# justinkay/aldi

Hardware: AMD Instinct MI355X
Metric: images/sec (student+teacher ALDI step), R50-FPN 1333x800 (higher is better)
Workload: dtype bf16

## Files before the change

### aldi_amd/csrc/elementwise.hip

```cpp
#include "common.h"
#include <stdlib.h>

namespace {

template <typename T>
__global__ void dgrad_weights_kernel(const float* __restrict__ w, const float* __restrict__ scale, T* __restrict__ wt,
                                     int Cout, int KH, int KW, int Cin) {
    long total = (long)Cout * KH * KW * Cin;
    for (long i = blockIdx.x * (long)blockDim.x + threadIdx.x; i < total; i += (long)gridDim.x * blockDim.x) {
        int co = (int)(i % Cout);
        long r = i / Cout;
        int kw = (int)(r % KW); r /= KW;
        int kh = (int)(r % KH);
        int ci = (int)(r / KH);
        float v = w[(((long)co * KH + (KH - 1 - kh)) * KW + (KW - 1 - kw)) * Cin + ci];
        if (scale) v *= scale[co];
        Elem<T>::st(wt + i, v);
    }
}

template <typename T>
__global__ __launch_bounds__(256) void dgrad_weights_batch_kernel(const aldi_dgw_item* __restrict__ items, int n_items) {
    __shared__ float tl[32][33];
    const int tile = blockIdx.x;
// ... 502 lines not shown
        p[i] = w;
        if (pc) Elem<T>::st(pc + i, w);
    }
}

template <typename T>
__global__ void ema_kernel(float* __restrict__ t, const float* __restrict__ s, T* __restrict__ tc, long n, long nc, float one_minus_alpha, float alpha,
                           int copy_only) {
    const long n4 = ((reinterpret_cast<uintptr_t>(t) | reinterpret_cast<uintptr_t>(s)) & 15) == 0 ? n >> 2 : 0;
    for (long q = blockIdx.x * (long)blockDim.x + threadIdx.x; q < n4; q += (long)gridDim.x * blockDim.x) {
        const float4 sv = reinterpret_cast<const float4*>(s)[q];
        float4 v = sv;
        if (!copy_only) {
            const float4 tv = reinterpret_cast<const float4*>(t)[q];
            v.x = sv.x * one_minus_alpha + tv.x * alpha; v.y = sv.y * one_minus_alpha + tv.y * alpha;
            v.z = sv.z * one_minus_alpha + tv.z * alpha; v.w = sv.w * one_minus_alpha + tv.w * alpha;
        }
        reinterpret_cast<float4*>(t)[q] = v;
        if (tc) {
            const long i = q << 2;
            if (i < nc) Elem<T>::st(tc + i, v.x);
            if (i + 1 < nc) Elem<T>::st(tc + i + 1, v.y);
            if (i + 2 < nc) Elem<T>::st(tc + i + 2, v.z);
            if (i + 3 < nc) Elem<T>::st(tc + i + 3, v.w);
        }
    }
    for (long i = (n4 << 2) + blockIdx.x * (long)blockDim.x + threadIdx.x; i < n; i += (long)gridDim.x * blockDim.x) {
        float v = copy_only ? s[i] : s[i] * one_minus_alpha + t[i] * alpha;
        t[i] = v;
        if (tc && i < nc) Elem<T>::st(tc + i, v);
    }
}

__global__ void bn_fold_kernel(const float* __restrict__ w, const float* __restrict__ b, const float* __restrict__ mean,
                               const float* __restrict__ var, float* __restrict__ scale, float* __restrict__ shift, int C, float eps) {
    int i = blockIdx.x * blockDim.x + threadIdx.x;
    if (i < C) {
        float sc = w[i] * (1.0f / sqrtf(var[i] + eps));
        scale[i] = sc;
        shift[i] = b[i] - mean[i] * sc;
    }
}

static inline int nblocks(long n, int per = 256, int cap = 16384) {
    long b = (n + per - 1) / per;
    return (int)(b < 1 ? 1 : (b > cap ? cap : b));
}

}

#define DISPATCH_T(dtype, KERNEL, grid, block, st, ...)                                              \
    do {                                                                                             \
        if ((dtype) == ALDI_BF16) hipLaunchKernelGGL(KERNEL<bf16_t>, grid, block, 0, st, __VA_ARGS__); \
        else if ((dtype) == ALDI_F32) hipLaunchKernelGGL(KERNEL<float>, grid, block, 0, st, __VA_ARGS__); \
        else return aldi_set_error_msg(ALDI_ERR_ARG, #KERNEL ": bad dtype");                         \
        ALDI_CHECK_LAUNCH();                                                                         \
    } while (0)

extern "C" int aldi_stem_forward(const aldi_stem_args* a, aldi_stream_t stream) {
    if (!a || !a->img || !a->w || !a->y || a->N < 1 || a->N > ALDI_MAX_IMAGES) return aldi_set_error_msg(ALDI_ERR_ARG, "stem_forward: bad args");
    StemDev d;
    d.img = a->img; d.w = a->w; d.scale = a->scale; d.shift = a->shift; d.y = a->y;
    d.N = a->N; d.Hs = a->Hs; d.Ws = a->Ws; d.Hc = a->Hc; d.Wc = a->Wc;
    for (int i = 0; i < a->N; ++i) { d.h[i] = a->h[i]; d.wd[i] = a->w_img[i]; }
    for (int c = 0; c < 3; ++c) { d.mean[c] = a->mean[c]; d.inv_std[c] = 1.0f / a->std[c]; }
    dim3 grid(cdiv(a->Wc, 16), cdiv(a->Hc, 16), a->N);
// ... 134 lines not shown
extern "C" int aldi_sgd_step(float* p, const float* g, float* buf, void* p_compute, long n, float lr, float momentum, float weight_decay,
                             float grad_scale, int first_step, int dtype, aldi_stream_t stream) {
    if (!p || !g || !buf) return aldi_set_error_msg(ALDI_ERR_ARG, "sgd_step: null pointer");
    hipStream_t st = static_cast<hipStream_t>(stream);
    if (dtype == ALDI_BF16) hipLaunchKernelGGL(sgd_kernel<bf16_t>, dim3(nblocks(n)), dim3(256), 0, st, p, g, buf, (bf16_t*)p_compute, n, lr, momentum, weight_decay, grad_scale, first_step);
    else hipLaunchKernelGGL(sgd_kernel<float>, dim3(nblocks(n)), dim3(256), 0, st, p, g, buf, (float*)nullptr, n, lr, momentum, weight_decay, grad_scale, first_step);
    ALDI_CHECK_LAUNCH();
    return ALDI_OK;
}

extern "C" int aldi_sgd_step_dev(float* p, const float* g, float* buf, void* p_compute, long n, const float* hyper, int dtype, aldi_stream_t stream) {
    if (!p || !g || !buf || !hyper || n <= 0) return aldi_set_error_msg(ALDI_ERR_ARG, "sgd_step_dev: bad args");
    hipStream_t st = static_cast<hipStream_t>(stream);
    if (dtype == ALDI_BF16) hipLaunchKernelGGL(sgd_dev_kernel<bf16_t>, dim3(nblocks(n)), dim3(256), 0, st, p, g, buf, (bf16_t*)p_compute, n, hyper);
    else hipLaunchKernelGGL(sgd_dev_kernel<float>, dim3(nblocks(n)), dim3(256), 0, st, p, g, buf, (float*)nullptr, n, hyper);
    ALDI_CHECK_LAUNCH();
    return ALDI_OK;
}

extern "C" int aldi_ema_update(float* teacher, const float* student, void* teacher_compute, long n, long n_compute, double alpha, int copy_only, int dtype,
                               aldi_stream_t stream) {
    if (!teacher || !student) return aldi_set_error_msg(ALDI_ERR_ARG, "ema_update: null pointer");
    hipStream_t st = static_cast<hipStream_t>(stream);
    const float oma = (float)(1.0 - alpha);
    const float alpha_f = (float)alpha;
    const long nc = teacher_compute ? (n_compute < n ? n_compute : n) : 0;
    const int cap = aldi_tuning().ema_blocks > 0 ? aldi_tuning().ema_blocks : 16384;
    if (dtype == ALDI_BF16) hipLaunchKernelGGL(ema_kernel<bf16_t>, dim3(nblocks(n / 4 + 1, 256, cap)), dim3(256), 0, st, teacher, student, (bf16_t*)teacher_compute, n, nc, oma, alpha_f, copy_only);
    else hipLaunchKernelGGL(ema_kernel<float>, dim3(nblocks(n / 4 + 1, 256, cap)), dim3(256), 0, st, teacher, student, (float*)nullptr, n, 0L, oma, alpha_f, copy_only);
    ALDI_CHECK_LAUNCH();
    return ALDI_OK;
}

extern "C" int aldi_bn_fold(const float* w, const float* b, const float* mean, const float* var, float* scale, float* shift, int C, aldi_stream_t stream) {
    hipLaunchKernelGGL(bn_fold_kernel, dim3(cdiv(C, 256)), dim3(256), 0, static_cast<hipStream_t>(stream), w, b, mean, var, scale, shift, C, 1e-5f);
    ALDI_CHECK_LAUNCH();
    return ALDI_OK;
}

extern "C" int aldi_dgrad_weights_batch(const aldi_dgw_item* items, int n_items, int total_tiles, int dtype, aldi_stream_t stream) {
    if (!items || n_items <= 0 || total_tiles <= 0) return aldi_set_error_msg(ALDI_ERR_ARG, "dgrad_weights_batch: bad args");
    hipStream_t st = static_cast<hipStream_t>(stream);
    if (dtype == ALDI_BF16) hipLaunchKernelGGL(dgrad_weights_batch_kernel<bf16_t>, dim3(total_tiles), dim3(256), 0, st, items, n_items);
    else if (dtype == ALDI_F32) hipLaunchKernelGGL(dgrad_weights_batch_kernel<float>, dim3(total_tiles), dim3(256), 0, st, items, n_items);
    else return aldi_set_error_msg(ALDI_ERR_ARG, "dgrad_weights_batch: bad dtype");
    ALDI_CHECK_LAUNCH();
    return ALDI_OK;
}

extern "C" int aldi_dgrad_weights(const float* w_master, const float* scale, void* wt, int Cout, int KH, int KW, int Cin,
                                  int dtype, aldi_stream_t stream) {
    if (!w_master || !wt) return aldi_set_error_msg(ALDI_ERR_ARG, "dgrad_weights: null pointer");
    long total = (long)Cout * KH * KW * Cin;
    int blocks = (int)((total + 255) / 256);
    if (blocks > 8192) blocks = 8192;
    hipStream_t st = static_cast<hipStream_t>(stream);
    if (dtype == ALDI_BF16) hipLaunchKernelGGL(dgrad_weights_kernel<bf16_t>, dim3(blocks), dim3(256), 0, st, w_master, scale, (bf16_t*)wt, Cout, KH, KW, Cin);
    else hipLaunchKernelGGL(dgrad_weights_kernel<float>, dim3(blocks), dim3(256), 0, st, w_master, scale, (float*)wt, Cout, KH, KW, Cin);
    ALDI_CHECK_LAUNCH();
    return ALDI_OK;
}
```

### aldi_amd/engine.py

```python
from __future__ import annotations

import contextlib
import dataclasses
import inspect
import math
import os
from collections import OrderedDict
from typing import Dict, List, Optional, Sequence, Tuple

import torch

from . import ops
from .arch import FC_DIM, FPN_C, NUM_ANCHORS, POOL, STAGE_BLOCKS, Packed, ParamLayout, pad_to

PIXEL_MEAN = (103.530, 116.280, 123.675)
PIXEL_STD = (1.0, 1.0, 1.0)
ANCHOR_SIZES = (32, 64, 128, 256, 512)
ANCHOR_RATIOS = (0.5, 1.0, 2.0)
STRIDES = (4, 8, 16, 32, 64)
GMAX = 128
RPN_BATCH, RPN_POS_FRAC = 256, 0.5
ROI_BATCH, ROI_POS_FRAC = 512, 0.25
RPN_PRE = (2000, 1000)
RPN_POST = (1000, 1000)
# ... 23 lines not shown
            a, a2 = torch.randperm(n_)[:k_], torch.randperm(17)
            torch.manual_seed(12345)
            b, b2 = fast(n_, k_), torch.randperm(17)
            ok = ok and torch.equal(a, b) and torch.equal(a2, b2)
        torch.set_rng_state(saved)
        _FAST_RANDPERM = ok
    if _FAST_RANDPERM:
        return fast(n, k)
    return torch.randperm(n)[:k]


class Weights:

    def __init__(self, layout: ParamLayout, device, dtype: torch.dtype, trainable: bool):
        self.layout, self.device, self.dtype, self.trainable = layout, device, dtype, trainable
        L = layout
        self.master = torch.zeros(L.n_total, dtype=torch.float32, device=device)
        self.compute = self.master if dtype == torch.float32 else torch.zeros(L.n_weights, dtype=dtype, device=device)
        self.bn_scale = torch.zeros(max(L.bn_channels, 1), dtype=torch.float32, device=device)
        self.bn_shift = torch.zeros(max(L.bn_channels, 1), dtype=torch.float32, device=device)
        self._grad = None
        self._mom = None
        self.first_step = True
        self._wt: Dict[str, torch.Tensor] = {}
        self._wt_keys: List[str] = []
        self._wt_plan = None
        self.wt_epoch = 0
        self._neg1: Dict[int, torch.Tensor] = {}
        self._stem_pk, self._stem_name = None, None
        self.lazy_wt = False
        self._wt_dirty = False
        self._fold_names: List[str] = []
        self._fold_plan = None

    @property
    def grad(self) -> torch.Tensor:
        if self._grad is None:
            self._grad = torch.zeros(self.layout.n_train, dtype=torch.float32, device=self.device)
        return self._grad

    @property
    def mom(self) -> torch.Tensor:
        if self._mom is None:
            self._mom = torch.zeros(self.layout.n_train, dtype=torch.float32, device=self.device)
        return self._mom

    def w(self, name: str) -> torch.Tensor:
        p = self.layout.t[name]
        n = p.rows * p.kk * p.kk * p.cin
        return self.compute[p.w_off: p.w_off + n].view(p.wshape)

    def w_master(self, name: str) -> torch.Tensor:
        p = self.layout.t[name]
        n = p.rows * p.kk * p.kk * p.cin
        return self.master[p.w_off: p.w_off + n].view(p.wshape)

    def b(self, name: str) -> Optional[torch.Tensor]:
        p = self.layout.t[name]
        return self.master[p.b_off: p.b_off + p.rows] if p.bias else None

    def scale(self, name: str) -> Optional[torch.Tensor]:
        p = self.layout.t[name]
        return self.bn_scale[p.bn_off: p.bn_off + p.rows] if p.bn else None

    def shift(self, name: str) -> Optional[torch.Tensor]:
        p = self.layout.t[name]
# ... 42 lines not shown
        neg = key.endswith("-")
        key = key[:-1] if neg else key
        flat = key.endswith("@flat")
        name = key[:-len("@flat")] if flat else key
        w = self.w_master(name)
        if flat:
            w = w.view(w.shape[0], 1, 1, -1)
        return w, self._wt_scale(name, neg)

    def _wt_scale(self, name: str, negate: bool):
        if not negate:
            return self.scale(name)
        rows = self.layout.t[name].rows
        if rows not in self._neg1:
            self._neg1[rows] = torch.full((rows,), -1.0, dtype=torch.float32, device=self.device)
        return self._neg1[rows]

    def _refresh_wt(self):
        self._wt_dirty = False
        self._wt.clear()
        if not self._wt_keys:
            return
        if self._wt_plan is None:
            self._wt_plan = ops.DgradWeightsPlan([self._wt_source(key) for key in self._wt_keys], self.dtype)
        self._wt_plan.run()
        for key, o in zip(self._wt_keys, self._wt_plan.out):
            self._wt[key] = o

    def load_state_dict(self, sd: Dict[str, torch.Tensor]):
        missing = [k for k in self.layout.state_dict_keys() if k not in sd]
        if missing:
            raise KeyError(f"missing keys in state_dict: {missing[:5]}{'...' if len(missing) > 5 else ''}")
        self.master.copy_(self.layout.pack(sd).to(self.device))
        self.refresh()

    def state_dict(self) -> "OrderedDict[str, torch.Tensor]":
        return self.layout.unpack(self.master)

    def refresh(self, cast: bool = True):
        L = self.layout
        if L.bn_channels:
            b = L.bn_base
            c = L.bn_channels
            ops.bn_fold(self.master[b:b + c], self.master[b + c:b + 2 * c], self.master[b + 2 * c:b + 3 * c],
                        self.master[b + 3 * c:b + 4 * c], self.bn_scale, self.bn_shift, c)
        if self.dtype != torch.float32 and cast:
            ops.cast_from_f32(self.master[:L.n_weights], self.dtype, out=self.compute)
        if self._stem_pk is not None:
            ops.stem_pack_weights(self.w_master(self._stem_name), out=self._stem_pk)
        if self._fold_plan is not None:
            self._fold_plan.run()
        self._refresh_wt()

    def zero_grad(self):
        self.grad.zero_()
        self._gscale = 1.0

    def scale_grad(self, f: float):
        self._gscale = getattr(self, "_gscale", 1.0) * f

    def sgd_step(self, lr: float, momentum: float = 0.9, weight_decay: float = 1e-4, grad_scale: float = 1.0):
        n = self.layout.n_train
        ops.sgd_step(self.master, self.grad, self.mom, self.compute if self.dtype != torch.float32 else None, n, lr, momentum,
                     weight_decay, grad_scale * getattr(self, "_gscale", 1.0), self.first_step, self.dtype)
        self._after_sgd()

    def _after_sgd(self):
        self.first_step = False
        if self.lazy_wt:
            self._wt_dirty = True
        else:
            self._refresh_wt()

    def sgd_range_dev(self, lo: int, hi: int, hyper: torch.Tensor):
        hi = min(hi, self.layout.n_train)
        if hi > lo:
            ops.sgd_step_dev(self.master, self.grad, self.mom, self.compute if self.dtype != torch.float32 else None, lo, hi, hyper, self.dtype)

    def ema_from(self, student: "Weights", alpha: float, copy_only: bool):
        n = self.layout.n_total
        if self.dtype == torch.bfloat16:
            ops.ema_update(self.master, student.master, self.compute, n, alpha, copy_only, self.dtype, n_compute=self.layout.n_weights)
            self.refresh(cast=False)
        else:
            ops.ema_update(self.master, student.master, None, n, alpha, copy_only, torch.float32)
            self.refresh()


def make_anchors(shapes: Sequence[Tuple[int, int]], device, sizes: Sequence[float] = ANCHOR_SIZES) -> torch.Tensor:
    out = []
    for (h, w), size, stride in zip(shapes, sizes, STRIDES):
        cell = []
        for r in ANCHOR_RATIOS:
            area = size ** 2.0
            aw = math.sqrt(area / r)
            ah = r * aw
            cell.append([-aw / 2.0, -ah / 2.0, aw / 2.0, ah / 2.0])
        cell = torch.tensor(cell, dtype=torch.float32)
# ... 1259 lines not shown
```

### aldi_amd/ops.py

```python
from __future__ import annotations

import ctypes as C
import os
from typing import List, Optional, Sequence

import torch

from . import _lib as L


def dtype_code(t: torch.dtype) -> int:
    if t == torch.float32:
        return L.F32
    if t == torch.bfloat16:
        return L.BF16
    raise TypeError(f"unsupported dtype {t}")


def _p(t: Optional[torch.Tensor]):
    return None if t is None else t.data_ptr()


_RAW_STREAM = getattr(torch._C, "_cuda_getCurrentRawStream", None)

# ... 299 lines not shown
    L.call("aldi_subsample2", _p(x), _p(y), N, H, W_, Cc, 0, dtype_code(x.dtype), stream_ptr())
    return y


def subsample2_bwd(g_small: torch.Tensor, g_big: torch.Tensor) -> None:
    N, H, W_, Cc = g_big.shape
    L.call("aldi_subsample2", _p(g_small), _p(g_big), N, H, W_, Cc, 1, dtype_code(g_big.dtype), stream_ptr())


def upsample2_bwd(g: torch.Tensor, out: torch.Tensor, accumulate: bool) -> None:
    N, Hc, Wc, Cc = out.shape
    assert g.shape == (N, Hc * 2, Wc * 2, Cc)
    L.call("aldi_upsample2_bwd", _p(g), _p(out), N, Hc, Wc, Cc, int(accumulate), dtype_code(g.dtype), stream_ptr())


def upsample2_bwd_chain(g2: torch.Tensor, o3: torch.Tensor, o4: torch.Tensor, o5: torch.Tensor) -> None:
    N, H5, W5, Cc = o5.shape
    assert o4.shape == (N, H5 * 2, W5 * 2, Cc) and o3.shape == (N, H5 * 4, W5 * 4, Cc) and g2.shape == (N, H5 * 8, W5 * 8, Cc)
    L.call("aldi_upsample2_bwd_chain", _p(g2), _p(o3), _p(o4), _p(o5), N, H5, W5, Cc, dtype_code(g2.dtype), stream_ptr())


def add_f32(a: Optional[torch.Tensor], b: Optional[torch.Tensor], out: torch.Tensor, relu_src: Optional[torch.Tensor] = None) -> torch.Tensor:
    L.call("aldi_add_f32", _p(a), _p(b), _p(relu_src), _p(out), out.numel(), dtype_code(out.dtype), stream_ptr())
    return out


def cast_from_f32(src: torch.Tensor, dtype: torch.dtype, out: Optional[torch.Tensor] = None) -> torch.Tensor:
    if out is None:
        out = torch.empty(src.shape, dtype=dtype, device=src.device)
    L.call("aldi_cast_from_f32", _p(src), _p(out), src.numel(), dtype_code(dtype), stream_ptr())
    return out


def sgd_step(p, g, buf, p_compute, n, lr, momentum, weight_decay, grad_scale, first_step, dtype) -> None:
    L.call("aldi_sgd_step", _p(p), _p(g), _p(buf), _p(p_compute), n, lr, momentum, weight_decay, grad_scale, int(first_step),
           dtype_code(dtype), stream_ptr())


def sgd_step_dev(p, g, buf, p_compute, lo: int, hi: int, hyper: torch.Tensor, dtype) -> None:
    pc = None if p_compute is None else p_compute.data_ptr() + lo * p_compute.element_size()
    L.call("aldi_sgd_step_dev", p.data_ptr() + 4 * lo, g.data_ptr() + 4 * lo, buf.data_ptr() + 4 * lo, pc, hi - lo, _p(hyper), dtype_code(dtype), stream_ptr())


def ema_update(teacher, student, teacher_compute, n, alpha, copy_only, dtype, n_compute=None) -> None:
    nc = 0 if teacher_compute is None else (teacher_compute.numel() if n_compute is None else n_compute)
    L.call("aldi_ema_update", _p(teacher), _p(student), _p(teacher_compute), n, nc, alpha, int(copy_only), dtype_code(dtype), stream_ptr())


def bn_fold(w, b, mean, var, scale, shift, Cc) -> None:
    L.call("aldi_bn_fold", _p(w), _p(b), _p(mean), _p(var), _p(scale), _p(shift), Cc, stream_ptr())


def make_geom(shapes: Sequence[Sequence[int]], A: int, Cc: int) -> L.RpnGeom:
    g = L.RpnGeom()
    g.num_levels, g.A, g.C = len(shapes), A, Cc
    off = 0
    for i, (h, w) in enumerate(shapes):
        g.H[i], g.W[i], g.off[i] = h, w, off
        off += h * w * A
    for i in range(len(shapes), L.MAX_LEVELS + 1):
        g.off[i] = off
    return g


def ptrs(ts: Optional[Sequence[Optional[torch.Tensor]]]):
    if ts is None:
        return None
# ... 160 lines not shown
```

### aldi_amd/trainer.py

```python
from __future__ import annotations

import contextlib
import copy
import logging
import os
import time
import weakref
from typing import Callable, Dict, List, NamedTuple, Optional

from collections import OrderedDict

import torch
import torch.distributed as dist

from . import synthetic
from .dataloader import DeviceStrongAugLoader, SyntheticDetectionLoader, WeakStrongDataloader, device_strong_seed
from .distill import build_distiller
from .ema import EMA
from .model import build_aldi

DEBUG = False
debug_dict = {}


# ... 216 lines not shown
        for k, v in out.items():
            if row.keep(k):
                entries.append((f"{k}_{name}", v))
    kept = [(n_, v) for n_, v in entries if not isinstance(v, tuple)]
    masked = [(n_, v[0]) for n_, v in entries if isinstance(v, tuple)]
    vals = {}
    if kept:
        kv = (torch.stack([v for _, v in kept]) / accum).detach()
        vals.update({n_: kv[i] for i, (n_, _) in enumerate(kept)})
    if masked:
        mv = ((torch.stack([v for _, v in masked]) * 0.0) / accum).detach()
        vals.update({n_: mv[i] for i, (n_, _) in enumerate(masked)})
    for n_, _ in entries:
        loss_dict[n_] = loss_dict[n_] + vals[n_] if n_ in loss_dict else vals[n_]
    eng.backward_fused(c, scales)
    model._last_fused = c
    return loss_dict


def _num_classes(cfg) -> int:
    if cfg.MODEL.META_ARCHITECTURE == "DeformableDETR":
        return int(cfg.MODEL.DEFORMABLE_DETR.NUM_CLASSES)
    return int(cfg.MODEL.ROI_HEADS.NUM_CLASSES)


class EngineSGD:
    def __init__(self, model, lr, momentum=0.9, weight_decay=1e-4):
        self.model = model
        self.param_groups = [{"lr": lr, "momentum": momentum, "weight_decay": weight_decay}]

    def zero_grad(self, set_to_none: bool = False):
        self.model.weights.zero_grad()

    def step(self):
        W = self.model.weights
        if getattr(W, "_sgd_applied", False):
            W._sgd_applied = False
            W._after_sgd()
            return
        g = self.param_groups[0]
        W.sgd_step(g["lr"], g["momentum"], g["weight_decay"])

    def state_dict(self):
        W = self.model.weights
        return {"format": "aldi_amd.flat_sgd", "param_groups": [dict(g) for g in self.param_groups],
                "momentum_buffer": None if W._mom is None else W.mom.detach().cpu().clone(), "first_step": bool(W.first_step)}

    def load_state_dict(self, sd):
        W = self.model.weights
        if sd.get("format") != "aldi_amd.flat_sgd":
            logging.getLogger(__name__).warning("optimizer state of a foreign format: momentum restarts from zero")
            return
        for g, h in zip(self.param_groups, sd.get("param_groups", [])):
            g.update({k: v for k, v in h.items() if k in ("momentum", "weight_decay")})
        if sd.get("momentum_buffer") is not None:
            W.mom.copy_(sd["momentum_buffer"].to(W.mom.device))
        W.first_step = bool(sd.get("first_step", sd.get("momentum_buffer") is None))


class EngineAdamW:
    def __init__(self, model, lr, weight_decay=0.1, betas=(0.9, 0.999), lr_decay_rate=None, num_layers=12):
        self.model = model
        self.param_groups = [{"lr": lr, "weight_decay": weight_decay, "betas": betas}]
        self.lr_decay_rate, self.num_layers = lr_decay_rate, num_layers

    def zero_grad(self, set_to_none: bool = False):
        self.model.weights.zero_grad()

    def step(self):
        g = self.param_groups[0]
        kw = {}
        if self.lr_decay_rate is not None:
            kw = dict(lr_decay_rate=self.lr_decay_rate, num_layers=self.num_layers)
# ... 87 lines not shown
        self.last_loss_dict: Dict[str, float] = {}

    @property
    def _data_loader_iter(self):
        if self._data_loader_iter_obj is None:
            self._data_loader_iter_obj = iter(self.data_loader)
        return self._data_loader_iter_obj

    def run_step(self):
        if not self.model.training:
            raise AssertionError("[SimpleTrainer] model was changed to eval mode!")
        t0 = time.perf_counter()
        batch = self._fetch_batch()
        fetch_s = time.perf_counter() - t0
        clear_first = self.zero_grad_before_forward
        if clear_first and self._defers_zero_grad():
            self._zero_pending = True
        elif clear_first:
            self.optimizer.zero_grad()
        if self._defers_sgd():
            self._sgd_pending = True
        result = self.run_model(batch)
        self.__dict__.pop("_sgd_pending", None)
        fused = bool(getattr(self, "_fused_done", False))
        if isinstance(result, torch.Tensor):
            loss_dict, total = {"total_loss": result}, result
        else:
            loss_dict, total = result, (None if fused else sum(result.values()))
        if not clear_first and not fused:
            self.optimizer.zero_grad()
        self.do_backward(total)
        self.after_backward()
        self._write_metrics(loss_dict, fetch_s)
        self.optimizer.step()

    def run_model(self, data):
        return self.model(data)

    def _wants_lookahead(self) -> bool:
        return False

    def _fetch_batch(self):
        if not self._wants_lookahead():
            ahead = self.__dict__.pop("_ahead_batch", None)
            self._next_batch = None
            return ahead if ahead is not None else next(self._data_loader_iter)
        ahead = self.__dict__.pop("_ahead_batch", None)
        batch = ahead if ahead is not None else next(self._data_loader_iter)
        try:
            self._ahead_batch = next(self._data_loader_iter)
        except StopIteration:
            self._ahead_batch = None
        self._next_batch = self._ahead_batch
        return batch

    def _defers_zero_grad(self) -> bool:
        return False

    def _defers_sgd(self) -> bool:
        return False

    def do_backward(self, losses):
        losses.backward()

    def after_backward(self):
        if _data_parallel():
# ... 84 lines not shown
            return False
        chunks = [ls[i:i + bs] for i in range(0, len(ls), bs)]
        if do_distill:
            from .distill import HardDistiller
            from .helpers import foreign_hooks
            d = self.distiller
            if type(d) is not HardDistiller or uw is None or us is None or len(uw) != len(us) or len(us) == 0 or len(us) % bs:
                return False
            if any(foreign_hooks(m.module if hasattr(m, "module") else m, []) for m in (d.student, d.teacher)):
                return False
            chunks += [us[i:i + bs] for i in range(0, len(us), bs)]
        if sum(len(c_) for c_ in chunks) > 16:
            return False
        canvas = {(max(int(b["image"].shape[-2]) for b in c_), max(int(b["image"].shape[-1]) for b in c_)) for c_ in chunks}
        return len({((h + 31) // 32, (w + 31) // 32) for h, w in canvas}) == 1

    def _wants_lookahead(self) -> bool:
        from .engine import RCNN
        model = self.model.module if hasattr(self.model, "module") else self.model
        eng = getattr(model, "engine", None)
        return (bool(self.fused) and (bool(model.cfg.SOLVER.get("PIPELINE_PREFIX", False)) or os.environ.get("ALDI_PIPELINE_PREFIX") == "1") and os.environ.get("ALDI_PIPELINE_PREFIX") != "0"
                and os.environ.get("ALDI_FUSED_LEGACY", "0") != "1" and type(eng) is RCNN and eng.prefix_pipelinable())

    def _defers_zero_grad(self) -> bool:
        from .engine import RCNN
        model = self.model.module if hasattr(self.model, "module") else self.model
        return bool(self.fused) and os.environ.get("ALDI_FUSED_LEGACY", "0") != "1" and type(getattr(model, "engine", None)) is RCNN

    def _defers_sgd(self) -> bool:
        W = getattr(self.model, "weights", None)
        return (self._defers_zero_grad() and isinstance(self.optimizer, EngineSGD) and not _data_parallel() and W is not None
                and not W.first_step and os.environ.get("ALDI_SGD_IN_STEP", "0") == "1")

    def run_model(self, data):
        self._fused_done = False
        pending_ema = self.__dict__.pop("_pending_ema", None)
        if pending_ema is not None and not self._can_fuse(data):
            pending_ema[0].update_weights(self.model, pending_ema[1])
            pending_ema = None
        defer = self.__dict__.pop("_zero_pending", False)
        if defer and not self._can_fuse(data):
            self.optimizer.zero_grad()
            defer = False
        if self._can_fuse(data):
            self._fused_done = True
            if not self.zero_grad_before_forward:
                if self._defers_zero_grad():
                    defer = True
                else:
                    self.optimizer.zero_grad()
            eng = self.model.engine
            reducer = None
            if _data_parallel():
                from .reduce import BucketedReducer, resolve_exchange
                reducer = self._reducer = BucketedReducer(self.model.weights.grad, payload=str(self.model.cfg.SOLVER.get("GRAD_PAYLOAD", "fp32")),
                                                          exchange=resolve_exchange(self.model.cfg.SOLVER.get("GRAD_EXCHANGE", "auto")))
                eng.grad_ready = reducer.ready
            ok = False
            try:
                if os.environ.get("ALDI_FUSED_LEGACY", "0") == "1":
                    out = fused_run_model(self, *data)
                    ok = True
                    return out
                if getattr(self, "_fused_step", None) is None:
                    from .fused_step import FusedStep
                    self._fused_step = FusedStep(self)
                sgd = None
                if self.__dict__.pop("_sgd_pending", False) and reducer is None:
                    g_ = self.optimizer.param_groups[0]
                    sgd = (g_["lr"], g_["momentum"], g_["weight_decay"])
                out = self._fused_step.run(*data, ema=pending_ema, zero_grad=defer, reducer=reducer, sgd=sgd,
                                           next_data=self.__dict__.get("_next_batch") if self._wants_lookahead() else None)
                ok = True
                return out
            finally:
                eng.grad_ready = None
                if not ok:
                    self._reducer = None
        if self._can_fuse_detr(data):
            self._fused_done = True
            return fused_run_model_detr(self, *data)
        return run_model_labeled_unlabeled(self, *data)

    def do_backward(self, losses, override=False):
        if getattr(self, "_fused_done", False):
            return
        if self.backward_at_end or override:
            super().do_backward(losses)


class ALDIAMPTrainer(_ALDITrainer, AMPTrainer):
    pass


class ALDISimpleTrainer(_ALDITrainer, SimpleTrainer):
    pass


class DefaultTrainer:
    def __init__(self, cfg):
        self.cfg = cfg
        model = self.build_model(cfg)
        optimizer = self.build_optimizer(cfg, model)
        data_loader = self.build_train_loader(cfg)
        model = self.create_ddp_model(model, broadcast_buffers=False, cfg=cfg)
        self._trainer = self._create_trainer(cfg, model, data_loader, optimizer)
# ... 128 lines not shown
        total = cfg.SOLVER.IMS_PER_BATCH
        sizes = [int(total * r / sum(ratios)) for r in ratios]
        if sum(sizes) != total:
            raise AssertionError(f"sum(batch_sizes)={sum(sizes)} must equal total_batch_size={total}")
        share = {}
        for part, n in zip(contents, sizes):
            share[part] = max(share.get(part, 0), n)
        labeled_bs = max((n for part, n in share.items() if part.startswith("labeled")), default=0)
        unlabeled_bs = max((n for part, n in share.items() if part.startswith("unlabeled")), default=0)
        batch_contents = contents
        world = dist.get_world_size() if dist.is_available() and dist.is_initialized() else 1
        rank = dist.get_rank() if world > 1 else 0
        syn = cfg.get("SYNTHETIC", {})
        h, w = syn.get("HEIGHT", 800), syn.get("WIDTH", 1333)
        K = _num_classes(cfg)
        fixed = bool(syn.get("FIXED", False))
        labeled_loader = SyntheticDetectionLoader(labeled_bs // world, h, w, K, 1000 + 17 * rank, True, fixed=fixed) if labeled_bs > 0 else None
        unlabeled_loader = SyntheticDetectionLoader(unlabeled_bs // world, h, w, K, 2000 + 17 * rank, False, fixed=fixed) if unlabeled_bs > 0 else None
        if cfg.AUG.get("DEVICE_STRONG", False):
            from .aug import get_strong_augs
            base = max(int(cfg.SEED), 0)
            if labeled_loader is not None:
                labeled_loader = DeviceStrongAugLoader(labeled_loader, get_strong_augs(cfg, True) if "labeled_strong" in contents else None,
                                                       device_strong_seed(base, rank, True))
            if unlabeled_loader is not None:
                unlabeled_loader = DeviceStrongAugLoader(unlabeled_loader, get_strong_augs(cfg, False) if "unlabeled_strong" in contents else None,
                                                         device_strong_seed(base, rank, False))
        return WeakStrongDataloader(labeled_loader, unlabeled_loader, batch_contents)

    def before_step(self):
        super(ALDITrainer, self).before_step()
        if self.cfg.EMA.ENABLED:
            t = self._trainer
            if getattr(t, "fused", False) and os.environ.get("ALDI_FUSED_LEGACY", "0") != "1" and type(t.model.engine).__name__ == "RCNN":
                t._pending_ema = (self.ema, self.iter)
            else:
                self.ema.update_weights(t.model, self.iter)

    @classmethod
    def build_test_loader(cls, cfg, dataset_name):
        syn_ = cfg.get("SYNTHETIC", {})
        h, w = syn_.get("HEIGHT", 800), syn_.get("WIDTH", 1333)
        n, K = int(syn_.get("VAL_IMAGES", 8)), _num_classes(cfg)
        g = torch.Generator().manual_seed(4242)
        batches, records = [], []
        for i in range(n):
            img, inst = synthetic.make_image(h, w, int(torch.randint(5, 21, (1,), generator=g)), K, g)
            batches.append([{"image": img, "image_id": i, "height": h, "width": w}])
            records.append(dict(image_id=i, height=h, width=w,
                                annotations=[dict(bbox=b.tolist(), bbox_mode="XYXY_ABS", category_id=int(c))
                                             for b, c in zip(inst["gt_boxes"], inst["gt_classes"])]))
        return batches, records

    @classmethod
    def build_evaluator(cls, cfg, dataset_name, output_folder=None, dataset_dicts=None):
        from .evaluation import Detectron2COCOEvaluatorAdapter, DeviceCOCOEvaluator
        if output_folder is None:
            output_folder = os.path.join(cfg.OUTPUT_DIR, "inference")
        if cfg.TEST.get("DEVICE_EVAL", False):
            return DeviceCOCOEvaluator(dataset_name, dataset_dicts or [], _num_classes(cfg), output_dir=output_folder)
        return Detectron2COCOEvaluatorAdapter(dataset_name, dataset_dicts or [], _num_classes(cfg), output_dir=output_folder)

    @classmethod
    def test(cls, cfg, model, evaluators=None):
        from .evaluation import inference_on_dataset
        names = list(cfg.DATASETS.TEST) or ["synthetic_val"]
# ... 29 lines not shown
```

### include/aldi_hip.h

```cpp
#ifndef ALDI_HIP_H
#define ALDI_HIP_H
#include <stddef.h>
#include <stdint.h>

#ifdef __cplusplus
extern "C" {
#endif

typedef void* aldi_stream_t;

enum { ALDI_F32 = 0, ALDI_BF16 = 1 };
enum { ALDI_OK = 0, ALDI_ERR_HIP = -1, ALDI_ERR_ARG = -2 };

const char* aldi_last_error(void);
int aldi_version(void);
int aldi_noop(aldi_stream_t stream);

int aldi_set_tuning(const char* name, int value);
int aldi_get_tuning(const char* name, int* value);
int aldi_reset_tuning(void);
const char* aldi_last_dispatch(void);

typedef struct {
    const void* x;
// ... 66 lines not shown
} aldi_fold_item;
int aldi_fold_weights_batch(const aldi_fold_item* items, int n_items, int total_chunks, aldi_stream_t stream);

#define ALDI_MAX_IMAGES 16

typedef struct {
    const uint8_t* img;
    const float* w;
    const float* scale; const float* shift;
    void* y;
    int N, Hs, Ws, Hc, Wc;
    int h[ALDI_MAX_IMAGES], w_img[ALDI_MAX_IMAGES];
    float mean[3], std[3];
    int dtype;
} aldi_stem_args;
int aldi_stem_forward(const aldi_stem_args* a, aldi_stream_t stream);
int aldi_stem_pack_weights(const float* w, void* w_packed, aldi_stream_t stream);
int aldi_stem_pool_forward(const aldi_stem_args* a, const void* w_packed, void* y_pool, aldi_stream_t stream);

int aldi_maxpool3s2(const void* x, void* y, int N, int H, int W, int C, int dtype, aldi_stream_t stream);
int aldi_stage_images(const void* const* images, const int* heights, const int* widths, int n, int C, int Hs, int Ws, void* batch,
                      aldi_stream_t stream);
int aldi_subsample2(const void* x, void* y, int N, int H, int W, int C, int backward, int dtype, aldi_stream_t stream);
int aldi_upsample2_bwd(const void* g, void* out, int N, int Hc, int Wc, int C, int accumulate, int dtype, aldi_stream_t stream);
int aldi_upsample2_bwd_chain(const void* g2, void* o3, void* o4, void* o5, int N, int H5, int W5, int C, int dtype, aldi_stream_t stream);
int aldi_add_f32(const void* a, const float* b, const void* relu_src, void* out, long n, int dtype, aldi_stream_t stream);
int aldi_cast_from_f32(const float* src, void* dst, long n, int dtype, aldi_stream_t stream);

int aldi_sgd_step(float* p, const float* g, float* buf, void* p_compute, long n, float lr, float momentum, float weight_decay,
                  float grad_scale, int first_step, int dtype, aldi_stream_t stream);
int aldi_sgd_step_dev(float* p, const float* g, float* buf, void* p_compute, long n, const float* hyper, int dtype, aldi_stream_t stream);
int aldi_ema_update(float* teacher, const float* student, void* teacher_compute, long n, long n_compute, double alpha, int copy_only, int dtype,
                    aldi_stream_t stream);
int aldi_bn_fold(const float* w, const float* b, const float* mean, const float* var, float* scale, float* shift, int C, aldi_stream_t stream);

#define ALDI_MAX_LEVELS 5
typedef struct {
    int num_levels;
    int A;
    int C;
    int H[ALDI_MAX_LEVELS], W[ALDI_MAX_LEVELS];
    int off[ALDI_MAX_LEVELS + 1];
} aldi_rpn_geom;

int aldi_box_match(const float* boxes, long box_stride_n, const int* box_count, int L,
                   const float* gt_boxes, const int* gt_count, int Gmax, int N,
                   float lo, float hi, int allow_low_quality,
                   float* best_iou, int* best_idx, unsigned* gt_best_scratch, size_t gt_best_bytes, int* labels, aldi_stream_t stream);
size_t aldi_compact_labels_workspace(int L, int N);
int aldi_compact_labels(const int* labels, int L, int N, int bg_label, int* lists, int* counts, void* workspace, aldi_stream_t stream);
int aldi_rpn_apply_sample(int* labels, int L, int N, const int* lists, const int* sel, const int* nsel, int S, aldi_stream_t stream);
int aldi_rpn_loss(const aldi_rpn_geom* gm, float* const* head, float* const* grad, const float* anchors, const int* labels, const int* matched,
                  const float* gt_boxes, const int* gt_count, int Gmax, int N, float inv_norm, float grad_scale_cls, float grad_scale_loc,
                  float* loss2, aldi_stream_t stream);
size_t aldi_rpn_proposals_workspace(int N, int num_levels);
int aldi_rpn_proposals(const aldi_rpn_geom* gm, float* const* head, const float* anchors, const int* img_hw, int N,
                       int pre_nms_topk, int post_nms_topk, float nms_thresh, void* workspace,
                       float* out_boxes, float* out_scores, int* out_count, int* err_flag, aldi_stream_t stream);

size_t aldi_rpn_active_pixels_workspace(const aldi_rpn_geom* gm, int N);
int aldi_rpn_active_pixels(const aldi_rpn_geom* gm, float* const* grad_head, int N, int cap, int* idx, int* count, void* workspace,
                           int* err_flag, aldi_stream_t stream);
int aldi_rpn_sparse_gather(const aldi_rpn_geom* gm, float* const* grad_head, const void* const* hidden, const void* const* feat, int N, int Cf,
                           int cap, const int* idx, const int* count, void* G, void* Tm, void* X9, int dtype, aldi_stream_t stream);
int aldi_rpn_sparse_scatter(const aldi_rpn_geom* gm, void* const* gfeat, const void* Y, int N, int Cf, int cap, const int* idx,
                            const int* count, int dtype, int grad_dtype, aldi_stream_t stream);
// ... 196 lines not shown
```

Baseline: 498.0.

## Fuse SGD step with next iteration's teacher EMA update in one kernel

Adds a state_step kernel that applies SGD momentum to the student master weights, writes the bf16 compute copy, and immediately applies the EMA lerp (or copy) into the teacher master and teacher bf16 copy in the same pass. The trainer rides the next iteration's EMA tick on the optimizer step when the fused path ran, then skips the separate EMA update in before_step. This removes a second full pass over the student weights and one extra kernel launch per iteration. In exchange it adds cross-iteration bookkeeping (tick_applied_for) and guards for eval, checkpoint and last-iteration boundaries.

```diff
diff --git a/aldi_amd/csrc/elementwise.hip b/aldi_amd/csrc/elementwise.hip
--- a/aldi_amd/csrc/elementwise.hip
+++ b/aldi_amd/csrc/elementwise.hip
@@ -558,6 +558,43 @@
     }
 }
 
+template <typename T>
+__global__ __launch_bounds__(256) void state_step_kernel(float* __restrict__ p, float* __restrict__ g, float* __restrict__ buf, T* __restrict__ pc,
+                                                         float* __restrict__ t, T* __restrict__ tc, long n_train, long n_weights, long n_total,
+                                                         float lr, float mu, float wd, float gscale, int first, float one_minus_alpha, float alpha,
+                                                         int copy_only, int clear_grad) {
+    const long n4 = n_total >> 2;
+    for (long q = blockIdx.x * (long)blockDim.x + threadIdx.x; q < n4; q += (long)gridDim.x * blockDim.x) {
+        const long i = q << 2;
+        float w[4];
+        load4(p + i, w);
+        if (i < n_train) {
+            float gv[4], b[4];
+            load4(g + i, gv);
+            if (!first) load4(buf + i, b);
+#pragma unroll
+            for (int k = 0; k < 4; ++k) {
+                const float d = gv[k] * gscale + wd * w[k];
+                b[k] = first ? d : mu * b[k] + d;
+                w[k] = w[k] - lr * b[k];
+            }
+            store4(buf + i, b);
+            store4(p + i, w);
+            store4(pc + i, w);
+            if (clear_grad) *reinterpret_cast<float4*>(g + i) = make_float4(0.f, 0.f, 0.f, 0.f);
+        }
+        float v[4] = {w[0], w[1], w[2], w[3]};
+        if (!copy_only) {
+            float tv[4];
+            load4(t + i, tv);
+#pragma unroll
+            for (int k = 0; k < 4; ++k) v[k] = w[k] * one_minus_alpha + tv[k] * alpha;
+        }
+        store4(t + i, v);
+        if (i < n_weights) store4(tc + i, v);
+    }
+}
+
 __global__ void bn_fold_kernel(const float* __restrict__ w, const float* __restrict__ b, const float* __restrict__ mean,
                                const float* __restrict__ var, float* __restrict__ scale, float* __restrict__ shift, int C, float eps) {
     int i = blockIdx.x * blockDim.x + threadIdx.x;
@@ -758,6 +795,25 @@
     return ALDI_OK;
 }
 
+extern "C" int aldi_state_step(float* p, float* g, float* buf, void* p_compute, float* teacher, void* teacher_compute, long n_train, long n_weights,
+                               long n_total, float lr, float momentum, float weight_decay, float grad_scale, int first_step, double alpha, int copy_only,
+                               int clear_grad, int dtype, aldi_stream_t stream) {
+    if (!p || !g || !buf || !p_compute || !teacher || !teacher_compute) return aldi_set_error_msg(ALDI_ERR_ARG, "state_step: null pointer");
+    if (dtype != ALDI_BF16) return aldi_set_error_msg(ALDI_ERR_ARG, "state_step: bf16 compute copies only");
+    if (n_train < 0 || n_train > n_weights || n_weights > n_total || n_total <= 0 || ((n_train | n_weights | n_total) & 3))
+        return aldi_set_error_msg(ALDI_ERR_ARG, "state_step: need 0 <= n_train <= n_weights <= n_total, each a multiple of 4");
+    if (((reinterpret_cast<uintptr_t>(p) | reinterpret_cast<uintptr_t>(g) | reinterpret_cast<uintptr_t>(buf) | reinterpret_cast<uintptr_t>(teacher)) & 15) ||
+        ((reinterpret_cast<uintptr_t>(p_compute) | reinterpret_cast<uintptr_t>(teacher_compute)) & 7))
+        return aldi_set_error_msg(ALDI_ERR_ARG, "state_step: buffers must be 16-byte aligned (compute copies: 8)");
+    const float oma = (float)(1.0 - alpha);
+    const float alpha_f = (float)alpha;
+    hipLaunchKernelGGL(state_step_kernel<bf16_t>, dim3(nblocks(n_total >> 2)), dim3(256), 0, static_cast<hipStream_t>(stream), p, g, buf, (bf16_t*)p_compute,
+                       teacher, (bf16_t*)teacher_compute, n_train, n_weights, n_total, lr, momentum, weight_decay, grad_scale, first_step, oma, alpha_f,
+                       copy_only, clear_grad);
+    ALDI_CHECK_LAUNCH();
+    return ALDI_OK;
+}
+
 extern "C" int aldi_bn_fold(const float* w, const float* b, const float* mean, const float* var, float* scale, float* shift, int C, aldi_stream_t stream) {
     hipLaunchKernelGGL(bn_fold_kernel, dim3(cdiv(C, 256)), dim3(256), 0, static_cast<hipStream_t>(stream), w, b, mean, var, scale, shift, C, 1e-5f);
     ALDI_CHECK_LAUNCH();
diff --git a/aldi_amd/engine.py b/aldi_amd/engine.py
--- a/aldi_amd/engine.py
+++ b/aldi_amd/engine.py
@@ -79,6 +79,7 @@
         self._wt_dirty = False
         self._fold_names: List[str] = []
         self._fold_plan = None
+        self.tick_applied_for = None
 
     @property
     def grad(self) -> torch.Tensor:
@@ -187,6 +188,7 @@
         if missing:
             raise KeyError(f"missing keys in state_dict: {missing[:5]}{'...' if len(missing) > 5 else ''}")
         self.master.copy_(self.layout.pack(sd).to(self.device))
+        self.tick_applied_for = None
         self.refresh()
 
     def state_dict(self) -> "OrderedDict[str, torch.Tensor]":
@@ -219,6 +221,20 @@
         ops.sgd_step(self.master, self.grad, self.mom, self.compute if self.dtype != torch.float32 else None, n, lr, momentum,
                      weight_decay, grad_scale * getattr(self, "_gscale", 1.0), self.first_step, self.dtype)
         self._after_sgd()
+
+    def sgd_ema_step(self, teacher: "Weights", alpha: float, copy_only: bool, lr: float, momentum: float = 0.9, weight_decay: float = 1e-4,
+                     clear_grad: bool = False):
+        L = self.layout
+        T = teacher.layout
+        if self.dtype != torch.bfloat16 or teacher.dtype != torch.bfloat16 or (L.n_train, L.n_weights, L.n_total) != (T.n_train, T.n_weights, T.n_total):
+            raise ValueError("sgd_ema_step: student and teacher must be bf16 models of the same flat layout")
+        ops.sgd_step(self.master, self.grad, self.mom, self.compute, L.n_train, lr, momentum, weight_decay, getattr(self, "_gscale", 1.0),
+                     self.first_step, self.dtype, teacher=teacher.master, teacher_compute=teacher.compute, n_weights=L.n_weights,
+                     n_total=L.n_total, alpha=alpha, copy_only=copy_only, clear_grad=clear_grad)
+        if clear_grad:
+            self._gscale = 1.0
+        self._after_sgd()
+        teacher.refresh(cast=False)
 
     def _after_sgd(self):
         self.first_step = False
diff --git a/aldi_amd/ops.py b/aldi_amd/ops.py
--- a/aldi_amd/ops.py
+++ b/aldi_amd/ops.py
@@ -355,7 +355,12 @@
     return out
 
 
-def sgd_step(p, g, buf, p_compute, n, lr, momentum, weight_decay, grad_scale, first_step, dtype) -> None:
+def sgd_step(p, g, buf, p_compute, n, lr, momentum, weight_decay, grad_scale, first_step, dtype, *, teacher=None, teacher_compute=None,
+             n_weights=None, n_total=None, alpha=None, copy_only=False, clear_grad=False) -> None:
+    if teacher is not None:
+        L.call("aldi_state_step", _p(p), _p(g), _p(buf), _p(p_compute), _p(teacher), _p(teacher_compute), n, n_weights, n_total, lr, momentum,
+               weight_decay, grad_scale, int(first_step), float(alpha), int(copy_only), int(clear_grad), dtype_code(dtype), stream_ptr())
+        return
     L.call("aldi_sgd_step", _p(p), _p(g), _p(buf), _p(p_compute), n, lr, momentum, weight_decay, grad_scale, int(first_step),
            dtype_code(dtype), stream_ptr())
 
diff --git a/aldi_amd/state_step.py b/aldi_amd/state_step.py
--- /dev/null
+++ b/aldi_amd/state_step.py
@@ -0,0 +1,18 @@
+import os
+
+
+def enabled() -> bool:
+    return os.environ.get("ALDI_STATE_STEP", "1") != "0"
+
+
+def tick_may_ride(it: int, max_iter: int, eval_period: int = 0, checkpoint_period: int = 0) -> bool:
+    if it + 1 >= max_iter:
+        return False
+    for period in (eval_period, checkpoint_period):
+        if period and period > 0 and (it + 1) % period == 0:
+            return False
+    return True
+
+
+def tick_mode(it: int, start_iter: int) -> str:
+    return "copy" if it <= start_iter else "lerp"
diff --git a/aldi_amd/trainer.py b/aldi_amd/trainer.py
--- a/aldi_amd/trainer.py
+++ b/aldi_amd/trainer.py
@@ -272,13 +272,18 @@
     def zero_grad(self, set_to_none: bool = False):
         self.model.weights.zero_grad()
 
-    def step(self):
+    def step(self, tick=None):
         W = self.model.weights
         if getattr(W, "_sgd_applied", False):
             W._sgd_applied = False
             W._after_sgd()
             return
         g = self.param_groups[0]
+        if tick is not None:
+            teacher, alpha, copy_only, it_next = tick
+            W.sgd_ema_step(teacher, alpha, copy_only, g["lr"], g["momentum"], g["weight_decay"])
+            teacher.tick_applied_for = it_next
+            return
         W.sgd_step(g["lr"], g["momentum"], g["weight_decay"])
 
     def state_dict(self):
@@ -432,6 +437,9 @@
         self.do_backward(total)
         self.after_backward()
         self._write_metrics(loss_dict, fetch_s)
+        self._optimizer_step()
+
+    def _optimizer_step(self):
         self.optimizer.step()
 
     def run_model(self, data):
@@ -582,8 +590,24 @@
         return (self._defers_zero_grad() and isinstance(self.optimizer, EngineSGD) and not _data_parallel() and W is not None
                 and not W.first_step and os.environ.get("ALDI_SGD_IN_STEP", "0") == "1")
 
+    def _optimizer_step(self):
+        from .engine import RCNN
+        from .state_step import tick_mode
+        ride = self.__dict__.pop("_ride_tick", None)
+        ran_fused = self.__dict__.pop("_fused_step_ran", False)
+        W = getattr(self.model, "weights", None)
+        if ride is not None and ran_fused and type(self.optimizer) is EngineSGD and not getattr(W, "_sgd_applied", False):
+            ema, it_next = ride
+            T = getattr(ema.model, "weights", None)
+            if (type(getattr(self.model, "engine", None)) is RCNN and type(getattr(ema.model, "engine", None)) is RCNN and W is not None and T is not None
+                    and W.dtype == torch.bfloat16 and T.dtype == torch.bfloat16):
+                self.optimizer.step(tick=(T, ema.alpha, tick_mode(it_next, ema.start_iter) == "copy", it_next))
+                return
+        self.optimizer.step()
+
     def run_model(self, data):
         self._fused_done = False
+        self._fused_step_ran = False
         pending_ema = self.__dict__.pop("_pending_ema", None)
         if pending_ema is not None and not self._can_fuse(data):
             pending_ema[0].update_weights(self.model, pending_ema[1])
@@ -622,6 +646,7 @@
                 out = self._fused_step.run(*data, ema=pending_ema, zero_grad=defer, reducer=reducer, sgd=sgd,
                                            next_data=self.__dict__.get("_next_batch") if self._wants_lookahead() else None)
                 ok = True
+                self._fused_step_ran = True
                 return out
             finally:
                 eng.grad_ready = None
@@ -816,6 +841,17 @@
         super(ALDITrainer, self).before_step()
         if self.cfg.EMA.ENABLED:
             t = self._trainer
+            from . import state_step
+            T = getattr(self.ema.model, "weights", None)
+            applied = getattr(T, "tick_applied_for", None)
+            if T is not None:
+                T.tick_applied_for = None
+            t.__dict__.pop("_ride_tick", None)
+            if state_step.enabled() and state_step.tick_may_ride(self.iter, self.max_iter, int(self.cfg.TEST.EVAL_PERIOD or 0),
+                                                                 int(self.cfg.SOLVER.get("CHECKPOINT_PERIOD", 0) or 0)):
+                t._ride_tick = (self.ema, self.iter + 1)
+            if applied is not None and applied == self.iter:
+                return
             if getattr(t, "fused", False) and os.environ.get("ALDI_FUSED_LEGACY", "0") != "1" and type(t.model.engine).__name__ == "RCNN":
                 t._pending_ema = (self.ema, self.iter)
             else:
diff --git a/include/aldi_hip.h b/include/aldi_hip.h
--- a/include/aldi_hip.h
+++ b/include/aldi_hip.h
@@ -122,6 +122,9 @@
 int aldi_sgd_step_dev(float* p, const float* g, float* buf, void* p_compute, long n, const float* hyper, int dtype, aldi_stream_t stream);
 int aldi_ema_update(float* teacher, const float* student, void* teacher_compute, long n, long n_compute, double alpha, int copy_only, int dtype,
                     aldi_stream_t stream);
+int aldi_state_step(float* p, float* g, float* buf, void* p_compute, float* teacher, void* teacher_compute, long n_train, long n_weights,
+                    long n_total, float lr, float momentum, float weight_decay, float grad_scale, int first_step, double alpha, int copy_only,
+                    int clear_grad, int dtype, aldi_stream_t stream);
 int aldi_bn_fold(const float* w, const float* b, const float* mean, const float* var, float* scale, float* shift, int C, aldi_stream_t stream);
 
 #define ALDI_MAX_LEVELS 5
```

Result: no change. 496.8, median of 3 (-0.2%).
